# borgor/ripcurrents

Measured on AMD Instinct MI355X. Metric: frames/sec dense Farneback flow @1080p, higher is better.
Workload: dtype f32

## Files before the change

### ripcurrents_amd/csrc/flow_iter_kernels.hip

```cpp

#include <cstdlib>

#include "rc_device.h"

#define RC_ITER_BATCH 3
#define RC_RR_D 3

#ifdef RC_EXACT_BUILD
#define RC_FLOW_NS rc_flow_exact
#else
#define RC_FLOW_NS rc_flow_fast
#endif
namespace RC_FLOW_NS {

__device__ __forceinline__ float2 rc_flow_in(const RcIterArgs& a, const float2* fin, int gx, int gy) {
    if (a.in_mode == 0) return make_float2(0.f, 0.f);
    if (a.in_mode == 1) return fin[(size_t)gy * a.w + gx];
    float ax, ay;
    int sx = rc_src_x(gx, a.up_scale_x, a.fin_w, ax);
    int sx1 = min(sx + 1, a.fin_w - 1);
    int sy = rc_src_y(gy, a.up_scale_y, ay);
    int sy0 = rc_clampi(sy, 0, a.fin_h - 1), sy1 = rc_clampi(sy + 1, 0, a.fin_h - 1);
    const float2* S0 = fin + (size_t)sy0 * a.fin_w;
    const float2* S1 = fin + (size_t)sy1 * a.fin_w;
// ... 454 lines not shown
        const int g4 = idx % (TW / 4), row = (idx / (TW / 4)) % CH, c = idx / (CH * (TW / 4));
        const float4* vp = (const float4*)(V + c * CH * VP + row * VP + 4 * g4);
        float v[4 * NQ];
#pragma unroll
        for (int q = 0; q < NQ; q++) {
            float4 t = vp[q];
            v[4 * q] = t.x; v[4 * q + 1] = t.y; v[4 * q + 2] = t.z; v[4 * q + 3] = t.w;
        }
        float o[4];
#pragma unroll
        for (int p = 0; p < 4; p++) {
            float s = v[M_ + p] * a.win.k[0];
#pragma unroll
            for (int i = 1; i <= M_; i++) s += a.win.k[i] * (v[M_ + p - i] + v[M_ + p + i]);
            o[p] = s;
        }
        *(float4*)(G + c * RING * MP + row * TW + 4 * g4) = make_float4(o[0], o[1], o[2], o[3]);
    }
    __syncthreads();
    for (int px = tid; px < CH * TW; px += NT) {
        const int row = px / TW, lx = px - row * TW;
        const int gx = tx0 + lx, gy = Y + row;
        double g[5];
#pragma unroll
        for (int c = 0; c < 5; c++) g[c] = G[c * RING * MP + px];
        if (gx < a.w && gy < yend) *(float2*)(fout + (size_t)gy * a.fout_step + (size_t)gx * 8) = rc_solve(g);
    }
    __syncthreads();
}

template <int M_, int NT, int BATCH>
__global__ __launch_bounds__(NT) void k_flow_iter_sweep(RcIterArgs a) {
    using S = RcSweep<M_>;
    constexpr int CH = S::CH, MW = S::MW, MP = S::MP, RING = S::RING, TW = S::TW;
    extern __shared__ __align__(16) float smf[];
    float* ring = smf;
    float* V = smf + 5 * RING * MP;
    const int tid = threadIdx.x;
    const int z = blockIdx.y;
    const int strip = blockIdx.x % a.tiles_x, seg = blockIdx.x / a.tiles_x;
    const int tx0 = strip * TW, y0 = seg * a.th;
    const int w = a.w, h = a.h;
    const int yend = min(y0 + a.th, h);
    const size_t s0 = (size_t)((a.slot0 + z * a.zstep) % a.nslots) * a.R_slot_stride;
    const size_t s1 = (size_t)((a.slot1 + z * a.zstep) % a.nslots) * a.R_slot_stride;
    const float4* RA0 = a.RA + s0;  const float* RB0 = a.RB + s0;
    const float4* RA1 = a.RA + s1;  const float* RB1 = a.RB + s1;
    const float2* fin = a.fin ? a.fin + (size_t)z * a.fin_pair_stride : nullptr;
    char* fout = a.fout + (size_t)z * a.fout_pair_stride;

    auto matrices_rows = [&](int r0, int nrows) {
        const int n = nrows * MW;
        for (int base = tid; base < n; base += NT * BATCH) {
            float2 d[BATCH];
            int gxs[BATCH], gys[BATCH];
#pragma unroll
            for (int q = 0; q < BATCH; q++) {
                const int idx = min(base + q * NT, n - 1);
                const int j = idx / MW, lx = idx - j * MW;
                gxs[q] = rc_clampi(tx0 - M_ + lx, 0, w - 1);
                gys[q] = rc_clampi(r0 + j, 0, h - 1);
                d[q] = rc_flow_in(a, fin, gxs[q], gys[q]);
            }
            RcM5 v[BATCH];
#pragma unroll
            for (int q = 0; q < BATCH; q++)
                v[q] = rc_matrices(RA0, RB0, RA1, RB1, gxs[q], gys[q], w, h, d[q].x, d[q].y);
#pragma unroll
            for (int q = 0; q < BATCH; q++) {
                const int idx = base + q * NT;
                if (idx < n) {
                    const int j = idx / MW, lx = idx - j * MW;
                    const int slot = (r0 + j - (y0 - M_)) % RING;
                    float* mp = ring + slot * MP + lx;
                    mp[0] = v[q].m0;
                    mp[RING * MP] = v[q].m1;
                    mp[2 * RING * MP] = v[q].m2;
                    mp[3 * RING * MP] = v[q].m3;
                    mp[4 * RING * MP] = v[q].m4;
                }
            }
        }
    };
    matrices_rows(y0 - M_, 2 * M_);
    const int nsteps = (yend - y0 + CH - 1) / CH;
    for (int s = 0; s < nsteps; s++) {
        matrices_rows(y0 + M_ + CH * s, CH);
        __syncthreads();
        const int Y = y0 + CH * s;
        switch (s % (RING / CH)) {
            case 0: rc_sweep_bc<M_, NT, 0>(a, ring, V, tid, tx0, Y, yend, fout); break;
            case 1: rc_sweep_bc<M_, NT, CH>(a, ring, V, tid, tx0, Y, yend, fout); break;
            case 2: rc_sweep_bc<M_, NT, 2 * CH>(a, ring, V, tid, tx0, Y, yend, fout); break;
            default: if constexpr (RING / CH > 3) rc_sweep_bc<M_, NT, 3 * CH>(a, ring, V, tid, tx0, Y, yend, fout); break;
        }
    }
}

template <int M, int NT, int BATCH>
static void launch_iter_sweep(RcIterArgs a, int pairs, hipStream_t s) {
    using S = RcSweep<M>;
    static_assert(S::RING / S::CH <= 4, "step dispatch covers four ring phases");
    RC_ALLOW_LDS((k_flow_iter_sweep<M, NT, BATCH>), S::LDS);
    a.tw = S::TW;
    a.tiles_x = (a.w + S::TW - 1) / S::TW;
    const int want = 4 * 512;
    int segs = (want + a.tiles_x * pairs - 1) / (a.tiles_x * pairs);
    int rs = (a.h + segs - 1) / segs;
    rs = ((rs + S::CH - 1) / S::CH) * S::CH;
    if (rs < 32) rs = 32;
    a.th = rs;
    a.tiles_y = (a.h + rs - 1) / rs;
    hipLaunchKernelGGL((k_flow_iter_sweep<M, NT, BATCH>), dim3(a.tiles_x * a.tiles_y, pairs, 1), dim3(NT), S::LDS, s, a);
}

#define RC_W3_THREADS 512
template <int IN_MODE, int GAUSS_>
__global__ __launch_bounds__(RC_W3_THREADS) void k_flow_iter_w3(RcIterArgs a) {
    constexpr int TW = 64, TH = 16, MW = TW + 2, MH = TH + 2, MP = MW | 1;
    constexpr int NITEMS = MW * MH, NIT = (NITEMS + RC_W3_THREADS - 1) / RC_W3_THREADS;
    extern __shared__ __align__(16) float smf[];
    float* Ms = smf;
    const int tid = threadIdx.x;
    const int z = blockIdx.y;
    const int t = a.xcd_remap ? rc_xcd_remap(blockIdx.x, a.tiles_x * a.tiles_y) : (int)blockIdx.x;
    const int tx0 = (t % a.tiles_x) * TW, ty0 = (t / a.tiles_x) * TH;
    const int w = a.w, h = a.h;
    const size_t s0 = (size_t)((a.slot0 + z * a.zstep) % a.nslots) * a.R_slot_stride;
    const size_t s1 = (size_t)((a.slot1 + z * a.zstep) % a.nslots) * a.R_slot_stride;
    const float4* __restrict__ RA0 = a.RA + s0;  const float* __restrict__ RB0 = a.RB + s0;
    const float4* __restrict__ RA1 = a.RA + s1;  const float* __restrict__ RB1 = a.RB + s1;
    const float2* __restrict__ fin = a.fin + (size_t)z * a.fin_pair_stride;
    char* fout = a.fout + (size_t)z * a.fout_pair_stride;

    int gx[NIT], gy[NIT];
#pragma unroll
    for (int q = 0; q < NIT; q++) {
        int idx = min(tid + q * RC_W3_THREADS, NITEMS - 1);
        int ly = idx / MW, lx = idx - ly * MW;
        gx[q] = rc_clampi(tx0 - 1 + lx, 0, w - 1);
        gy[q] = rc_clampi(ty0 - 1 + ly, 0, h - 1);
    }
    float dx[NIT], dy[NIT];
    if constexpr (IN_MODE == 0) {
#pragma unroll
        for (int q = 0; q < NIT; q++) dx[q] = dy[q] = 0.f;
    } else if constexpr (IN_MODE == 1) {
        float2 d[NIT];
#pragma unroll
        for (int q = 0; q < NIT; q++) d[q] = fin[(size_t)gy[q] * w + gx[q]];
#pragma unroll
        for (int q = 0; q < NIT; q++) { dx[q] = d[q].x; dy[q] = d[q].y; }
    } else {
        float2 p00[NIT], p01[NIT], p10[NIT], p11[NIT];
        float ax[NIT], ay[NIT];
#pragma unroll
        for (int q = 0; q < NIT; q++) {
            int sx = rc_src_x(gx[q], a.up_scale_x, a.fin_w, ax[q]);
            int sx1 = min(sx + 1, a.fin_w - 1);
            int sy = rc_src_y(gy[q], a.up_scale_y, ay[q]);
            int sy0 = rc_clampi(sy, 0, a.fin_h - 1), sy1 = rc_clampi(sy + 1, 0, a.fin_h - 1);
            const float2* S0 = fin + (size_t)sy0 * a.fin_w;
            const float2* S1 = fin + (size_t)sy1 * a.fin_w;
            p00[q] = S0[sx]; p01[q] = S0[sx1]; p10[q] = S1[sx]; p11[q] = S1[sx1];
        }
#pragma unroll
        for (int q = 0; q < NIT; q++) {
            float a0 = 1.f - ax[q], a1 = ax[q], b0 = 1.f - ay[q], b1 = ay[q];
            float r0x = p00[q].x * a0 + p01[q].x * a1, r1x = p10[q].x * a0 + p11[q].x * a1;
            float r0y = p00[q].y * a0 + p01[q].y * a1, r1y = p10[q].y * a0 + p11[q].y * a1;
            dx[q] = (r0x * b0 + r1x * b1) * a.up_mul;
            dy[q] = (r0y * b0 + r1y * b1) * a.up_mul;
        }
    }
    float4 A0[NIT];
    float B0[NIT];
    RcGather gt[NIT];
#pragma unroll
    for (int q = 0; q < NIT; q++) {
        size_t p0 = (size_t)gy[q] * w + gx[q];
        A0[q] = RA0[p0];
        B0[q] = RB0[p0];
        rc_r0_prep(A0[q], B0[q]);
        rc_gather_issue(gt[q], RA1, RB1, gx[q], gy[q], dx[q], dy[q], w, h);
    }
#pragma unroll
    for (int q = 0; q < NIT; q++) {
        RcM5 v = rc_matrices_reg(A0[q], B0[q], gt[q], dx[q], dy[q], gx[q], gy[q], w, h);
        int idx = tid + q * RC_W3_THREADS;
        if (idx < NITEMS) {
            int ly = idx / MW, lx = idx - ly * MW;
            float* mp = Ms + ly * MP + lx;
            mp[0] = v.m0;
            mp[MH * MP] = v.m1;
            mp[2 * MH * MP] = v.m2;
            mp[3 * MH * MP] = v.m3;
            mp[4 * MH * MP] = v.m4;
        }
    }
    __syncthreads();

    constexpr int RPT = TH / (RC_W3_THREADS / TW);
    const int lx = tid % TW, r0 = (tid / TW) * RPT;
    const int ox = tx0 + lx;
    float g[RPT][5];
#pragma unroll
    for (int c = 0; c < 5; c++) {
        const float* mc = Ms + c * MH * MP + r0 * MP + lx;
        float col[3][RPT + 2];
#pragma unroll
        for (int j = 0; j < 3; j++)
#pragma unroll
            for (int r = 0; r < RPT + 2; r++) col[j][r] = mc[r * MP + j];
#pragma unroll
        for (int r = 0; r < RPT; r++) {
            float v[3];
#pragma unroll
            for (int j = 0; j < 3; j++) {
                if (GAUSS_) v[j] = col[j][r + 1] * a.win.k[0] + (col[j][r + 2] + col[j][r]) * a.win.k[1];
                else v[j] = col[j][r + 1] + (col[j][r + 2] + col[j][r]);
            }
            if (GAUSS_) g[r][c] = v[1] * a.win.k[0] + a.win.k[1] * (v[0] + v[2]);
            else g[r][c] = (v[1] + v[0]) + v[2];
        }
    }
    if (ox < w) {
#pragma unroll
        for (int r = 0; r < RPT; r++) {
            int oy = ty0 + r0 + r;
            if (oy < h)
                *(float2*)(fout + (size_t)oy * a.fout_step + (size_t)ox * 8) =
                    rc_solve3(g[r], GAUSS_ ? 1e-3f : (float)a.win.box_eps);
        }
    }
}

template <int IN_MODE, int G>
static void launch_w3(RcIterArgs a, int pairs, hipStream_t s) {
    a.tw = 64; a.th = 16;
    a.tiles_x = (a.w + 63) / 64; a.tiles_y = (a.h + 15) / 16;
    size_t lds = sizeof(float) * 5 * 18 * 67;
    hipLaunchKernelGGL((k_flow_iter_w3<IN_MODE, G>), dim3(a.tiles_x * a.tiles_y, pairs, 1), dim3(RC_W3_THREADS), lds, s, a);
}

template <int WW, int WH, int WP = WW>
__device__ __forceinline__ void rc_gather_window(RcGather& g, const float4* LA, const float* LB, int ox, int oy,
                                                 const float4* __restrict__ RA1, const float* __restrict__ RB1,
                                                 int gx, int gy, float dx, float dy, int w, int h) {
    float fx = gx + dx, fy = gy + dy;
    int x1 = (int)floorf(fx), y1 = (int)floorf(fy);
    g.fx = fx - x1;
    g.fy = fy - y1;
    g.inside = (unsigned)x1 < (unsigned)(w - 1) && (unsigned)y1 < (unsigned)(h - 1);
    const int wx = x1 - ox, wy = y1 - oy;
    if (g.inside && (unsigned)wx < (unsigned)(WW - 1) && (unsigned)wy < (unsigned)(WH - 1)) {
        const int i = wy * WP + wx;
        g.q00 = LA[i]; g.q01 = LA[i + 1]; g.q10 = LA[i + WP]; g.q11 = LA[i + WP + 1];
        g.e00 = LB[i]; g.e01 = LB[i + 1]; g.e10 = LB[i + WP]; g.e11 = LB[i + WP + 1];
    } else {
        const size_t p = g.inside ? (size_t)y1 * w + x1 : (size_t)gy * w + gx;
        const size_t pw = g.inside ? (size_t)w : 0, p1 = g.inside ? 1 : 0;
        g.q00 = RA1[p]; g.q01 = RA1[p + p1]; g.q10 = RA1[p + pw]; g.q11 = RA1[p + pw + p1];
        g.e00 = RB1[p]; g.e01 = RB1[p + p1]; g.e10 = RB1[p + pw]; g.e11 = RB1[p + pw + p1];
    }
}

__device__ __forceinline__ void rc_hsum3_dpp(float (&g)[5], const float (&V)[5]) {
    float t0, t1, t2, t3, t4;
    asm("s_nop 1\n\t"
        "v_add_f32_dpp %5, %10, %10 wave_shr:1 row_mask:0xf bank_mask:0xf bound_ctrl:1\n\t"
        "v_add_f32_dpp %6, %11, %11 wave_shr:1 row_mask:0xf bank_mask:0xf bound_ctrl:1\n\t"
        "v_add_f32_dpp %7, %12, %12 wave_shr:1 row_mask:0xf bank_mask:0xf bound_ctrl:1\n\t"
        "v_add_f32_dpp %8, %13, %13 wave_shr:1 row_mask:0xf bank_mask:0xf bound_ctrl:1\n\t"
        "v_add_f32_dpp %9, %14, %14 wave_shr:1 row_mask:0xf bank_mask:0xf bound_ctrl:1\n\t"
        "v_add_f32_dpp %0, %10, %5 wave_shl:1 row_mask:0xf bank_mask:0xf bound_ctrl:1\n\t"
        "v_add_f32_dpp %1, %11, %6 wave_shl:1 row_mask:0xf bank_mask:0xf bound_ctrl:1\n\t"
        "v_add_f32_dpp %2, %12, %7 wave_shl:1 row_mask:0xf bank_mask:0xf bound_ctrl:1\n\t"
        "v_add_f32_dpp %3, %13, %8 wave_shl:1 row_mask:0xf bank_mask:0xf bound_ctrl:1\n\t"
        "v_add_f32_dpp %4, %14, %9 wave_shl:1 row_mask:0xf bank_mask:0xf bound_ctrl:1"
        : "=&v"(g[0]), "=&v"(g[1]), "=&v"(g[2]), "=&v"(g[3]), "=&v"(g[4]),
          "=&v"(t0), "=&v"(t1), "=&v"(t2), "=&v"(t3), "=&v"(t4)
        : "v"(V[0]), "v"(V[1]), "v"(V[2]), "v"(V[3]), "v"(V[4]));
}


__device__ __forceinline__ void rc_hpair_dpp(float (&s)[5], const float (&V)[5]) {
    float t0, t1, t2, t3, t4;
    asm("s_nop 1\n\t"
        "v_mov_b32_dpp %5, %10 wave_shr:1 row_mask:0xf bank_mask:0xf bound_ctrl:1\n\t"
        "v_mov_b32_dpp %6, %11 wave_shr:1 row_mask:0xf bank_mask:0xf bound_ctrl:1\n\t"
        "v_mov_b32_dpp %7, %12 wave_shr:1 row_mask:0xf bank_mask:0xf bound_ctrl:1\n\t"
        "v_mov_b32_dpp %8, %13 wave_shr:1 row_mask:0xf bank_mask:0xf bound_ctrl:1\n\t"
        "v_mov_b32_dpp %9, %14 wave_shr:1 row_mask:0xf bank_mask:0xf bound_ctrl:1\n\t"
        "v_add_f32_dpp %0, %10, %5 wave_shl:1 row_mask:0xf bank_mask:0xf bound_ctrl:1\n\t"
        "v_add_f32_dpp %1, %11, %6 wave_shl:1 row_mask:0xf bank_mask:0xf bound_ctrl:1\n\t"
        "v_add_f32_dpp %2, %12, %7 wave_shl:1 row_mask:0xf bank_mask:0xf bound_ctrl:1\n\t"
        "v_add_f32_dpp %3, %13, %8 wave_shl:1 row_mask:0xf bank_mask:0xf bound_ctrl:1\n\t"
        "v_add_f32_dpp %4, %14, %9 wave_shl:1 row_mask:0xf bank_mask:0xf bound_ctrl:1"
        : "=&v"(s[0]), "=&v"(s[1]), "=&v"(s[2]), "=&v"(s[3]), "=&v"(s[4]),
          "=&v"(t0), "=&v"(t1), "=&v"(t2), "=&v"(t3), "=&v"(t4)
        : "v"(V[0]), "v"(V[1]), "v"(V[2]), "v"(V[3]), "v"(V[4]));
}

template <int GAUSS_, int NIT, int MW, int NG>
__device__ __forceinline__ void rc_rr_flows(const float (&m)[NIT][5], const float* XR, int grp, int x,
                                            const RcWindow& win, float2 (&f)[NIT]) {
    const int gu = max(grp - 1, 0), gd = min(grp + 1, NG - 1);
    const int bu = (int)__umul24((unsigned)gu, 10u * MW) + x, bd = (int)__umul24((unsigned)gd, 10u * MW) + x;
    float up[5], dn[5];
#pragma unroll
    for (int c = 0; c < 5; c++) {
        up[c] = XR[bu + (5 + c) * MW];
        dn[c] = XR[bd + c * MW];
    }
    float V[NIT][5];
#pragma unroll
    for (int q = 0; q < NIT; q++)
#pragma unroll
        for (int c = 0; c < 5; c++) {
            float u = q > 0 ? m[q - 1][c] : up[c], d = q < NIT - 1 ? m[q + 1][c] : dn[c];
            if (GAUSS_) V[q][c] = m[q][c] * win.k[0] + (d + u) * win.k[1];
            else V[q][c] = m[q][c] + (d + u);
        }
#pragma unroll
    for (int q = 0; q < NIT; q++) {
        float g[5];
        if (GAUSS_) {
            float lr[5];
            rc_hpair_dpp(lr, V[q]);
#pragma unroll
            for (int c = 0; c < 5; c++) g[c] = V[q][c] * win.k[0] + win.k[1] * lr[c];
        } else {
            rc_hsum3_dpp(g, V[q]);
        }
        f[q] = rc_solve3(g, GAUSS_ ? 1e-3f : (float)win.box_eps);
    }
}

template <int NIT, int MW>
__device__ __forceinline__ void rc_rr_exchange(const float (&m)[NIT][5], float* XR, int grp, int x) {
    const int b = (int)__umul24((unsigned)grp, 10u * MW) + x;
#pragma unroll
    for (int c = 0; c < 5; c++) {
        XR[b + c * MW] = m[0][c];
        XR[b + (5 + c) * MW] = m[NIT - 1][c];
    }
}

template <int IN_MODE, int NIT, int MW, int MH, bool INTERIOR = false>
__device__ __forceinline__ void rc_rr_flow_in(const RcIterArgs& a, const float2* __restrict__ fin, int tx0, int ty0,
                                              int gxo, const int (&gys)[NIT], float (&dx)[NIT], float (&dy)[NIT]) {
    const int w = a.w, h = a.h;
    if constexpr (IN_MODE == 0) {
#pragma unroll
        for (int q = 0; q < NIT; q++) dx[q] = dy[q] = 0.f;
    } else if constexpr (IN_MODE == 1) {
        float2 d[NIT];
#pragma unroll
        for (int q = 0; q < NIT; q++) d[q] = INTERIOR ? fin[(unsigned)(gys[q] * w + gxo)] : fin[(size_t)gys[q] * w + gxo];
#pragma unroll
        for (int q = 0; q < NIT; q++) { dx[q] = d[q].x; dy[q] = d[q].y; }
    } else if ((NIT % 2 == 0) && a.up_exact2 && (INTERIOR || (ty0 - 2 >= 0 && ty0 - 2 + MH <= h))) {
        constexpr int NR = NIT / 2 + 2;
        int sx = (gxo - 1) >> 1;
        float ax = (gxo & 1) ? 0.25f : 0.75f;
        if (!INTERIOR) {
            if (sx < 0) { ax = 0.f; sx = 0; }
            if (sx >= a.fin_w - 1) { ax = 0.f; sx = a.fin_w - 1; }
        }
        const int sx1 = min(sx + 1, a.fin_w - 1);
        const int rb = (gys[0] - 1) >> 1;
        float2 t0[NR], t1[NR];
        typedef float rc_f4a8 __attribute__((ext_vector_type(4), aligned(8)));
        const bool cols_plain = INTERIOR || (tx0 - 2 >= 1 && tx0 - 2 + MW <= w && ((tx0 - 2 + MW - 2) >> 1) + 1 <= a.fin_w - 1);
        if (INTERIOR) {
            unsigned co = (unsigned)(__mul24(rb, a.fin_w) + sx);
#pragma unroll
            for (int j = 0; j < NR; j++) {
                const rc_f4a8 v = *(const rc_f4a8*)(fin + co);
                t0[j] = make_float2(v.x, v.y); t1[j] = make_float2(v.z, v.w);
                co += (unsigned)a.fin_w;
            }
        } else if (cols_plain) {
#pragma unroll
            for (int j = 0; j < NR; j++) {
                const float2* S = fin + (size_t)rc_clampi(rb + j, 0, a.fin_h - 1) * a.fin_w;
                const rc_f4a8 v = *(const rc_f4a8*)(S + sx);
                t0[j] = make_float2(v.x, v.y); t1[j] = make_float2(v.z, v.w);
            }
        } else {
#pragma unroll
            for (int j = 0; j < NR; j++) {
                const float2* S = fin + (size_t)rc_clampi(rb + j, 0, a.fin_h - 1) * a.fin_w;
                t0[j] = S[sx]; t1[j] = S[sx1];
            }
        }
        const float a0 = 1.f - ax, a1 = ax;
        float hx[NR], hy[NR];
#pragma unroll
        for (int j = 0; j < NR; j++) {
            hx[j] = t0[j].x * a0 + t1[j].x * a1;
            hy[j] = t0[j].y * a0 + t1[j].y * a1;
        }
#pragma unroll
        for (int q = 0; q < NIT; q++) {
            const int j0 = (q + 1) >> 1;
            const float b1 = (q & 1) ? 0.25f : 0.75f, b0 = 1.f - b1;
            dx[q] = (hx[j0] * b0 + hx[j0 + 1] * b1) * a.up_mul;
            dy[q] = (hy[j0] * b0 + hy[j0 + 1] * b1) * a.up_mul;
        }
    } else {
        float2 p00[NIT], p01[NIT], p10[NIT], p11[NIT];
        float ax, ay[NIT];
        int sx, sys[NIT];
        if (a.up_exact2) {
            sx = (gxo - 1) >> 1;
            ax = (gxo & 1) ? 0.25f : 0.75f;
            if (sx < 0) { ax = 0.f; sx = 0; }
            if (sx >= a.fin_w - 1) { ax = 0.f; sx = a.fin_w - 1; }
#pragma unroll
            for (int q = 0; q < NIT; q++) { sys[q] = (gys[q] - 1) >> 1; ay[q] = (gys[q] & 1) ? 0.25f : 0.75f; }
        } else {
            sx = rc_src_x(gxo, a.up_scale_x, a.fin_w, ax);
#pragma unroll
            for (int q = 0; q < NIT; q++) sys[q] = rc_src_y(gys[q], a.up_scale_y, ay[q]);
        }
        const int sx1 = min(sx + 1, a.fin_w - 1);
#pragma unroll
        for (int q = 0; q < NIT; q++) {
            int sy = sys[q];
            int sy0 = rc_clampi(sy, 0, a.fin_h - 1), sy1 = rc_clampi(sy + 1, 0, a.fin_h - 1);
            const float2* S0 = fin + (size_t)sy0 * a.fin_w;
            const float2* S1 = fin + (size_t)sy1 * a.fin_w;
            p00[q] = S0[sx]; p01[q] = S0[sx1]; p10[q] = S1[sx]; p11[q] = S1[sx1];
        }
#pragma unroll
        for (int q = 0; q < NIT; q++) {
            float a0 = 1.f - ax, a1 = ax, b0 = 1.f - ay[q], b1 = ay[q];
            float r0x = p00[q].x * a0 + p01[q].x * a1, r1x = p10[q].x * a0 + p11[q].x * a1;
            float r0y = p00[q].y * a0 + p01[q].y * a1, r1y = p10[q].y * a0 + p11[q].y * a1;
            dx[q] = (r0x * b0 + r1x * b1) * a.up_mul;
            dy[q] = (r0y * b0 + r1y * b1) * a.up_mul;
        }
    }
}


__device__ __forceinline__ void rc_lds_barrier() { asm volatile("s_waitcnt lgkmcnt(0)\n\ts_barrier" ::: "memory"); }
__device__ __forceinline__ void rc_all_barrier() { asm volatile("s_waitcnt vmcnt(0) lgkmcnt(0)\n\ts_barrier" ::: "memory"); }

constexpr bool rc_recip_exact(int nt, int wp) {
    const unsigned r = (65536u + wp - 1) / wp;
    for (int t = 0; t < nt; t++)
        if ((int)((t * r) >> 16) != t / wp) return false;
    return true;
}

__device__ __forceinline__ void rc_glds16_s(const void* base, unsigned voff, uint32_t lds_wave_addr) {
    asm volatile("s_mov_b32 m0, %2\n\ts_nop 0\n\tglobal_load_lds_dwordx4 %0, %1" ::"v"(voff), "s"(base), "s"(lds_wave_addr) : "memory");
}
__device__ __forceinline__ void rc_glds4_s(const void* base, unsigned voff, uint32_t lds_wave_addr) {
    asm volatile("s_mov_b32 m0, %2\n\ts_nop 0\n\tglobal_load_lds_dword %0, %1" ::"v"(voff), "s"(base), "s"(lds_wave_addr) : "memory");
}

template <bool INTERIOR, int NT, int WP, int WN, int NWL>
__device__ __forceinline__ void rc_rrc_issue_window(const float4* __restrict__ RA1, const float* __restrict__ RB1,
                                                    uint32_t lds_a, uint32_t lds_b, int tid, int ox, int oy, int w, int h) {
    constexpr int QY = NT / WP, QX = NT % WP;
    const int wave_base = __builtin_amdgcn_readfirstlane(tid & ~63);
    static_assert(rc_recip_exact(NT, WP), "tid / WP by multiply and shift must be exact for every thread");
    int wy = (int)(__umul24((unsigned)tid, (65536u + WP - 1) / WP) >> 16), wx = tid - (int)__umul24((unsigned)wy, (unsigned)WP);
    int off = __mul24(oy + wy, w) + ox + wx;
#pragma unroll
    for (int q = 0; q < NWL; q++) {
        bool ok = (q + 1) * NT <= WN || tid + q * NT < WN;
        if (!INTERIOR) ok = ok && (unsigned)(ox + wx) < (unsigned)w && (unsigned)(oy + wy) < (unsigned)h;
        const unsigned p = ok ? (unsigned)off : 0u;
        if (q * NT + wave_base < WN) {
            rc_glds16_s(RA1, p << 4, lds_a + (uint32_t)(q * NT + wave_base) * 16u);
            rc_glds4_s(RB1, p << 2, lds_b + (uint32_t)(q * NT + wave_base) * 4u);
        }
        wx += QX; wy += QY; off += QY * w + QX;
        if (wx >= WP) { wx -= WP; wy += 1; off += w - WP; }
    }
}

template <bool INTERIOR, int NIT, int WW, int WH, int WP>
__device__ __forceinline__ void rc_rr_matrices(float (&m)[NIT][5], const float4 (&A0)[NIT], const float (&B0)[NIT],
                                               const float (&dx)[NIT], const float (&dy)[NIT], const float4* LA,
                                               const float* LB, int ox, int oy, const float4* __restrict__ RA1,
                                               const float* __restrict__ RB1, int gxo, const int (&gys)[NIT], int w, int h) {
    if constexpr (!INTERIOR) {
#pragma unroll
        for (int q = 0; q < NIT; q++) {
            RcGather g;
            rc_gather_window<WW, WH, WP>(g, LA, LB, ox, oy, RA1, RB1, gxo, gys[q], dx[q], dy[q], w, h);
            RcM5 v = rc_matrices_reg(A0[q], B0[q], g, dx[q], dy[q], gxo, gys[q], w, h, true);
            m[q][0] = v.m0; m[q][1] = v.m1; m[q][2] = v.m2; m[q][3] = v.m3; m[q][4] = v.m4;
        }
    } else {
        unsigned far = 0;
#pragma unroll
        for (int q = 0; q < NIT; q++) {
            RcGather g;
            const float fx = gxo + dx[q], fy = gys[q] + dy[q];
            const float flx = floorf(fx), fly = floorf(fy);
            const int x1 = (int)flx, y1 = (int)fly;
            g.fx = fx - flx;
            g.fy = fy - fly;
            g.inside = true;
            const int wx = x1 - ox, wy = y1 - oy;
            const bool in_win = (unsigned)wx < (unsigned)(WW - 1) && (unsigned)wy < (unsigned)(WH - 1);
            far |= in_win ? 0u : 1u << q;
            const unsigned i = in_win ? __umul24((unsigned)wy, (unsigned)WP) + (unsigned)wx : 0u;
            const float4* pa = (const float4*)((const char*)LA + (i << 4));
            const float* pb = (const float*)((const char*)LB + (i << 2));
            g.q00 = pa[0]; g.q01 = pa[1]; g.q10 = pa[WP]; g.q11 = pa[WP + 1];
            g.e00 = pb[0]; g.e01 = pb[1]; g.e10 = pb[WP]; g.e11 = pb[WP + 1];
            RcM5 v = rc_matrices_reg(A0[q], B0[q], g, dx[q], dy[q], gxo, gys[q], w, h, false);
            m[q][0] = v.m0; m[q][1] = v.m1; m[q][2] = v.m2; m[q][3] = v.m3; m[q][4] = v.m4;
        }
        if (__builtin_expect(far != 0, 0)) {
#pragma unroll
            for (int q = 0; q < NIT; q++) {
                if (far >> q & 1) {
                    RcGather g;
                    rc_gather_issue(g, RA1, RB1, gxo, gys[q], dx[q], dy[q], w, h);
                    RcM5 v = rc_matrices_reg(A0[q], B0[q], g, dx[q], dy[q], gxo, gys[q], w, h, false);
                    m[q][0] = v.m0; m[q][1] = v.m1; m[q][2] = v.m2; m[q][3] = v.m3; m[q][4] = v.m4;
                }
            }
        }
    }
}

template <bool INTERIOR, int IN_MODE, int GAUSS_, int NIT, int D, int MW, int NG>
__device__ __forceinline__ void rc_rrc_body(const RcIterArgs& a, const int zb, const int ze, float* smf, const uint32_t lds0, const int tx0, const int ty0) {
    constexpr int NT = NG * MW, MH = NG * NIT;
    constexpr int WW = MW + 2 * D, WH = MH + 2 * D, WP = WW, WN = WP * WH, NWL = (WN + NT - 1) / NT;
    constexpr int WNP = (WN + 63) & ~63;
    constexpr int MP = MW + 1, PLANE = MH * MP;
    static_assert(5 * PLANE <= 5 * WNP, "border-block M1 planes alias the R1 window");
    float4* LA = (float4*)smf;
    float* LB = smf + 4 * WNP;
    float* XR = LB + WNP;
    float* Ms = smf;
    const uint32_t lds_a = lds0, lds_b = lds0 + 16u * WNP;
    const int w = a.w, h = a.h;
    const int ox = tx0 - 2 - D, oy = ty0 - 2 - D;
#define RC_RRC_COORDS(tid_)                                                         \
    const int x = (tid_) & (MW - 1), grp = (tid_) / MW, ly0 = grp * NIT;            \
    const int px = tx0 - 2 + x;                                                     \
    const int gxo = INTERIOR ? px : rc_clampi(px, 0, w - 1);                        \
    int gys[NIT];                                                                   \
    _Pragma("unroll") for (int q = 0; q < NIT; q++)                                 \
        gys[q] = INTERIOR ? ty0 - 2 + ly0 + q : rc_clampi(ty0 - 2 + ly0 + q, 0, h - 1);

    float4 A0[NIT];
    float B0[NIT];
    float dx[NIT], dy[NIT];
    {
        const int tid = threadIdx.x;
        RC_RRC_COORDS(tid)
        const size_t s0 = (size_t)((a.slot0 + zb * a.zstep) % a.nslots) * a.R_slot_stride;
        const size_t s1 = (size_t)((a.slot1 + zb * a.zstep) % a.nslots) * a.R_slot_stride;
        rc_rrc_issue_window<INTERIOR, NT, WP, WN, NWL>(a.RA + s1, a.RB + s1, lds_a, lds_b, tid, ox, oy, w, h);
#pragma unroll
        for (int q = 0; q < NIT; q++) {
            const unsigned p0 = (unsigned)(gys[q] * w + gxo);
            A0[q] = (a.RA + s0)[p0];
            B0[q] = (a.RB + s0)[p0];
            rc_r0_prep(A0[q], B0[q]);
        }
        rc_rr_flow_in<IN_MODE, NIT, MW, MH, INTERIOR>(a, a.fin + (size_t)zb * a.fin_pair_stride, tx0, ty0, gxo, gys, dx, dy);
    }

    for (int z = zb; z < ze; z++) {
        const size_t s1 = (size_t)((a.slot1 + z * a.zstep) % a.nslots) * a.R_slot_stride;
        const float4* __restrict__ RA1 = a.RA + s1;
        const float* __restrict__ RB1 = a.RB + s1;
        const bool more = z + 1 < ze;
        int tid = threadIdx.x;
        asm volatile("" : "+v"(tid));
        RC_RRC_COORDS(tid)
        rc_all_barrier();

        float m[NIT][5];
        rc_rr_matrices<INTERIOR, NIT, WW, WH, WP>(m, A0, B0, dx, dy, LA, LB, ox, oy, RA1, RB1, gxo, gys, w, h);
        rc_rr_exchange<NIT, MW>(m, XR, grp, x);
        rc_lds_barrier();

        {
            float2 f1[NIT];
            rc_rr_flows<GAUSS_, NIT, MW, NG>(m, XR, grp, x, a.win, f1);
            float f1x[NIT], f1y[NIT];
#pragma unroll
            for (int q = 0; q < NIT; q++) { f1x[q] = f1[q].x; f1y[q] = f1[q].y; }
            rc_rr_matrices<INTERIOR, NIT, WW, WH, WP>(m, A0, B0, f1x, f1y, LA, LB, ox, oy, RA1, RB1, gxo, gys, w, h);
        }
        if (more) {
#pragma unroll
            for (int q = 0; q < NIT; q++) {
                const int i = (int)__umul24((unsigned)(gys[q] - oy), (unsigned)WP) + (gxo - ox);
                A0[q] = LA[i];
                B0[q] = LB[i];
                rc_r0_prep(A0[q], B0[q]);
            }
        }
        rc_lds_barrier();
        if constexpr (!INTERIOR) {
#pragma unroll
            for (int q = 0; q < NIT; q++)
#pragma unroll
                for (int c = 0; c < 5; c++) Ms[c * PLANE + (ly0 + q) * MP + x] = m[q][c];
            rc_lds_barrier();
#pragma unroll
            for (int q = 0; q < NIT; q++) {
                const int py = ty0 - 2 + ly0 + q;
                if ((unsigned)px >= (unsigned)w || (unsigned)py >= (unsigned)h) {
                    const int cx = gxo - (tx0 - 2), cy = gys[q] - (ty0 - 2);
#pragma unroll
                    for (int c = 0; c < 5; c++) m[q][c] = Ms[c * PLANE + cy * MP + cx];
                }
            }
        }
        rc_rr_exchange<NIT, MW>(m, XR, grp, x);
        rc_lds_barrier();

        if (more) {
            const size_t n1 = (size_t)((a.slot1 + (z + 1) * a.zstep) % a.nslots) * a.R_slot_stride;
            rc_rrc_issue_window<INTERIOR, NT, WP, WN, NWL>(a.RA + n1, a.RB + n1, lds_a, lds_b, tid, ox, oy, w, h);
        }

        {
            char* fout = a.fout + (size_t)z * a.fout_pair_stride;
            float2 f2[NIT];
            rc_rr_flows<GAUSS_, NIT, MW, NG>(m, XR, grp, x, a.win, f2);
            if (x >= 2 && x < MW - 2 && (INTERIOR || px < w)) {
                unsigned so = (unsigned)(ty0 - 2 + ly0) * (unsigned)a.fout_step + (unsigned)px * 8u;
#pragma unroll
                for (int q = 0; q < NIT; q++) {
                    const int ly = ly0 + q, py = ty0 - 2 + ly;
                    if (ly >= 2 && ly < MH - 2 && (INTERIOR || py < h)) *(float2*)(fout + so) = f2[q];
                    so += (unsigned)a.fout_step;
                }
            }
        }
        if (more) rc_rr_flow_in<IN_MODE, NIT, MW, MH, INTERIOR>(a, a.fin + (size_t)(z + 1) * a.fin_pair_stride, tx0, ty0, gxo, gys, dx, dy);
    }
#undef RC_RRC_COORDS
}

template <int IN_MODE, int GAUSS_, int NIT, int D, int MINB, int MW, int NG>
__global__ __launch_bounds__(NG * MW, MINB) void k_flow_iter2_rrc(RcIterArgs a, RcChainPlan cp) {
    constexpr int MH = NG * NIT, TW = MW - 4, TH = MH - 4;
    extern __shared__ __align__(16) float smf[];
    const int zb = cp.ngroups ? cp.start[blockIdx.y] : (int)blockIdx.y, ze = cp.ngroups ? cp.start[blockIdx.y + 1] : zb + 1;
    const int t = a.xcd_remap ? rc_xcd_remap(blockIdx.x, a.tiles_x * a.tiles_y) : (int)blockIdx.x;
    const int tx0 = (t % a.tiles_x) * TW, ty0 = (t / a.tiles_x) * TH;
    const bool interior = tx0 - 2 >= 5 && tx0 - 2 + MW <= a.w - 5 && ty0 - 2 >= 5 && ty0 - 2 + MH <= a.h - 5;
    const uint32_t lds0 = (uint32_t)(uintptr_t)(__attribute__((address_space(3))) void*)smf;
    if (interior) rc_rrc_body<true, IN_MODE, GAUSS_, NIT, D, MW, NG>(a, zb, ze, smf, lds0, tx0, ty0);
    else rc_rrc_body<false, IN_MODE, GAUSS_, NIT, D, MW, NG>(a, zb, ze, smf, lds0, tx0, ty0);
}

template <int IN_MODE, int G, int NIT, int D, int MINB, int MW = 32, int NG = 8>
static void launch_rrc_t(RcIterArgs a, const RcChainPlan& cp, int pairs, hipStream_t s) {
    constexpr int MH = NG * NIT, TW = MW - 4, TH = MH - 4;
    a.tw = TW; a.th = TH;
    a.tiles_x = (a.w + TW - 1) / TW; a.tiles_y = (a.h + TH - 1) / TH;
    constexpr int WN = (MW + 2 * D) * (MH + 2 * D), WNP = (WN + 63) & ~63;
    const size_t lds = sizeof(float) * (5 * WNP + NG * 2 * 5 * MW);
    RC_ALLOW_LDS((k_flow_iter2_rrc<IN_MODE, G, NIT, D, MINB, MW, NG>), lds);
    hipLaunchKernelGGL((k_flow_iter2_rrc<IN_MODE, G, NIT, D, MINB, MW, NG>), dim3(a.tiles_x * a.tiles_y, cp.ngroups ? cp.ngroups : pairs, 1), dim3(NG * MW), lds, s, a, cp);
}

static void rc_chain_plan(const RcIterArgs& a, int pairs, long long tiles, RcChainPlan& cp) {
    cp.ngroups = 0;
    const bool chainable = a.chain > 1 && pairs > 1 && (a.slot0 + a.zstep) % a.nslots == a.slot1 % a.nslots;
    if (!chainable) return;
    int chain = a.chain;
    if (!(a.ablate & RC_ABL_FORCE_CHAIN))
        while (chain > 1 && tiles * pairs / chain < (a.chain_min_blocks > 0 ? a.chain_min_blocks : 4096)) chain >>= 1;
    if (chain <= 1) return;
    int n = 0, z = 0;
    cp.start[0] = 0;
    while (z < pairs) {
        int left = pairs - z, c = left > chain ? chain : (left + 1) / 2;
        if (n == RC_MAX_CHAIN_GROUPS - 1) c = left;
        z += c;
        cp.start[++n] = z;
    }
    cp.ngroups = n;
}

template <int IN_MODE, int G>
static void launch_w3x2(RcIterArgs a, int pairs, hipStream_t s) {
    const long long tiles = (long long)((a.w + 27) / 28) * ((a.h + 27) / 28), blocks = tiles * pairs;
    RcChainPlan cp;
    rc_chain_plan(a, pairs, tiles, cp);
    if (cp.ngroups) launch_rrc_t<IN_MODE, G, 4, RC_RR_D, 4>(a, cp, pairs, s);
    else if (blocks < 512) launch_rrc_t<IN_MODE, G, 2, 4, 6>(a, cp, pairs, s);
    else if (blocks < 1024) launch_rrc_t<IN_MODE, G, 3, 4, 5>(a, cp, pairs, s);
    else launch_rrc_t<IN_MODE, G, 4, RC_RR_D, 4>(a, cp, pairs, s);
}

int rc_flow_iter_can_fuse2(const RcIterArgs& a) { return a.win.m == 1 && a.solve && a.addr32; }

int rc_flow_iter2_r0_reads(const RcIterArgs& a, int pairs) {
    RcChainPlan cp;
    rc_chain_plan(a, pairs, (long long)((a.w + 27) / 28) * ((a.h + 27) / 28), cp);
    return cp.ngroups ? cp.ngroups : pairs;
}

int rc_flow_chain_groups(const RcIterArgs& a, int pairs, int* starts, int cap) {
    RcChainPlan cp;
    rc_chain_plan(a, pairs, (long long)((a.w + 27) / 28) * ((a.h + 27) / 28), cp);
    for (int i = 0; i <= cp.ngroups && i < cap; i++) starts[i] = cp.start[i];
    return cp.ngroups;
}

void rc_launch_flow_iter2(const RcIterArgs& a, int pairs, hipStream_t s) {
    const int g = a.win.gaussian ? 1 : 0;
    switch (a.in_mode * 2 + g) {
        case 0: launch_w3x2<0, 0>(a, pairs, s); break;
        case 1: launch_w3x2<0, 1>(a, pairs, s); break;
        case 2: launch_w3x2<1, 0>(a, pairs, s); break;
        case 3: launch_w3x2<1, 1>(a, pairs, s); break;
        case 4: launch_w3x2<2, 0>(a, pairs, s); break;
        default: launch_w3x2<2, 1>(a, pairs, s); break;
    }
}

static size_t iter_lds(int tw, int th, int m, bool two_buffers) {
    int MW = tw + 2 * m, MH = th + 2 * m, MP = MW | 1;
    return sizeof(float) * (5 * (size_t)MH * MP + (two_buffers ? 5 * (size_t)th * MP : 0));
}

template <int TW, int TH, int M, int G>
static void launch_iter_t(RcIterArgs a, int pairs, hipStream_t s) {
    size_t lds = iter_lds(TW, TH, M, M > 1);
    RC_ALLOW_LDS((k_flow_iter<TW, TH, M, G>), lds);
    a.tw = TW; a.th = TH;
    a.tiles_x = (a.w + TW - 1) / TW; a.tiles_y = (a.h + TH - 1) / TH;
    hipLaunchKernelGGL((k_flow_iter<TW, TH, M, G>), dim3(a.tiles_x * a.tiles_y, pairs, 1), dim3(RC_BLOCK), lds, s, a);
}

static void pick_runtime_tile(int m, int& tw, int& th) {
    static const int tiles[][2] = {{64, 16}, {32, 32}, {64, 8}, {32, 16}, {16, 16}, {16, 8}, {8, 8}};
    double best = -1;
    tw = 8; th = 8;
    for (auto& t : tiles) {
        size_t lds = iter_lds(t[0], t[1], m, true);
        if (lds > 150 * 1024) continue;
        double eff = (double)(t[0] * t[1]) / ((t[0] + 2 * m) * (t[1] + 2 * m));
        if (lds > 64 * 1024) eff *= 0.6;
        if (t[0] < 64) eff *= 0.95;
        if (eff > best) { best = eff; tw = t[0]; th = t[1]; }
    }
}

void rc_launch_flow_iter(const RcIterArgs& a, int pairs, hipStream_t s) {
    const int m = a.win.m, g = a.win.gaussian ? 1 : 0;
    if (m == 1 && a.solve) {
        switch (a.in_mode * 2 + g) {
            case 0: launch_w3<0, 0>(a, pairs, s); break;
            case 1: launch_w3<0, 1>(a, pairs, s); break;
            case 2: launch_w3<1, 0>(a, pairs, s); break;
            case 3: launch_w3<1, 1>(a, pairs, s); break;
            case 4: launch_w3<2, 0>(a, pairs, s); break;
            default: launch_w3<2, 1>(a, pairs, s); break;
        }
        return;
    }
    if (m == 1) { g ? launch_iter_t<64, 16, 1, 1>(a, pairs, s) : launch_iter_t<64, 16, 1, 0>(a, pairs, s); return; }
    if (a.solve) {
        if (m == 2) { g ? launch_iter_big<2, 1, 512>(a, pairs, s) : launch_iter_big<2, 0, 512>(a, pairs, s); return; }
        const long long work = (long long)a.w * a.h * pairs;
        if (g && (m == 5 || m == 10) && !(a.ablate & RC_ABL_TILE_WINDOW) &&
            ((a.ablate & RC_ABL_FORCE_SWEEP) || work >= (m == 10 ? 900000ll : 8000000ll))) {
            m == 5 ? launch_iter_sweep<5, 1024, 1>(a, pairs, s) : launch_iter_sweep<10, 1024, 1>(a, pairs, s);
            return;
        }
        if (m == 5) { g ? launch_iter_big<5, 1, 1024>(a, pairs, s) : launch_iter_big<5, 0, 1024>(a, pairs, s); return; }
        if (m == 10) { g ? launch_iter_big<10, 1, 1024, 64>(a, pairs, s) : launch_iter_big<10, 0, 1024, 64>(a, pairs, s); return; }
    }
    if (m == 2) { g ? launch_iter_t<64, 16, 2, 1>(a, pairs, s) : launch_iter_t<64, 16, 2, 0>(a, pairs, s); return; }
    if (m == 5) { g ? launch_iter_t<32, 32, 5, 1>(a, pairs, s) : launch_iter_t<32, 32, 5, 0>(a, pairs, s); return; }
    if (m == 10) { g ? launch_iter_t<32, 32, 10, 1>(a, pairs, s) : launch_iter_t<32, 32, 10, 0>(a, pairs, s); return; }
    RcIterArgs b = a;
    pick_runtime_tile(m, b.tw, b.th);
    b.tiles_x = (b.w + b.tw - 1) / b.tw; b.tiles_y = (b.h + b.th - 1) / b.th;
    size_t lds = iter_lds(b.tw, b.th, m, true);
    RC_ALLOW_LDS((k_flow_iter<0, 0, 0, 0>), lds);
    hipLaunchKernelGGL((k_flow_iter<0, 0, 0, 0>), dim3(b.tiles_x * b.tiles_y, pairs, 1), dim3(RC_BLOCK), lds, s, b);
}

}
```

Before: 20170.

## Pair top and bottom halo row-groups into one edge wave to skip dead rows

Reassigns row groups to waves so one wave per block (rotated by block index) holds the first and last row groups, which contain the halo rows; that wave skips the second-iteration matrix rebuild for halo-only rows and the output flow for both halo rows. The other waves handle the interior groups with remapped exchange offsets in LDS. This removes redundant compute on halo rows in every iteration. It adds a second specialization of the body (more code, separate edge/non-edge templates) and reversed row indexing for the odd half of the edge wave, which can cause divergence within that wave.

```diff
diff --git a/ripcurrents_amd/csrc/flow_iter_kernels.hip b/ripcurrents_amd/csrc/flow_iter_kernels.hip
--- a/ripcurrents_amd/csrc/flow_iter_kernels.hip
+++ b/ripcurrents_amd/csrc/flow_iter_kernels.hip
@@ -780,20 +780,18 @@
         : "v"(V[0]), "v"(V[1]), "v"(V[2]), "v"(V[3]), "v"(V[4]));
 }
 
-template <int GAUSS_, int NIT, int MW, int NG>
-__device__ __forceinline__ void rc_rr_flows(const float (&m)[NIT][5], const float* XR, int grp, int x,
+template <int GAUSS_, int NIT, int MW, int Q0>
+__device__ __forceinline__ void rc_rr_flows(const float (&m)[NIT][5], const float* XR, int bu, int bd,
                                             const RcWindow& win, float2 (&f)[NIT]) {
-    const int gu = max(grp - 1, 0), gd = min(grp + 1, NG - 1);
-    const int bu = (int)__umul24((unsigned)gu, 10u * MW) + x, bd = (int)__umul24((unsigned)gd, 10u * MW) + x;
     float up[5], dn[5];
 #pragma unroll
     for (int c = 0; c < 5; c++) {
-        up[c] = XR[bu + (5 + c) * MW];
+        up[c] = Q0 == 0 ? XR[bu + c * MW] : 0.f;
         dn[c] = XR[bd + c * MW];
     }
     float V[NIT][5];
 #pragma unroll
-    for (int q = 0; q < NIT; q++)
+    for (int q = Q0; q < NIT; q++)
 #pragma unroll
         for (int c = 0; c < 5; c++) {
             float u = q > 0 ? m[q - 1][c] : up[c], d = q < NIT - 1 ? m[q + 1][c] : dn[c];
@@ -801,7 +799,7 @@
             else V[q][c] = m[q][c] + (d + u);
         }
 #pragma unroll
-    for (int q = 0; q < NIT; q++) {
+    for (int q = Q0; q < NIT; q++) {
         float g[5];
         if (GAUSS_) {
             float lr[5];
@@ -815,13 +813,12 @@
     }
 }
 
-template <int NIT, int MW>
-__device__ __forceinline__ void rc_rr_exchange(const float (&m)[NIT][5], float* XR, int grp, int x) {
-    const int b = (int)__umul24((unsigned)grp, 10u * MW) + x;
+template <bool EDGE, int NIT, int MW>
+__device__ __forceinline__ void rc_rr_exchange(const float (&m)[NIT][5], float* XR, int b0, int b1) {
 #pragma unroll
     for (int c = 0; c < 5; c++) {
-        XR[b + c * MW] = m[0][c];
-        XR[b + (5 + c) * MW] = m[NIT - 1][c];
+        if (!EDGE) XR[b0 + c * MW] = m[0][c];
+        XR[b1 + c * MW] = m[NIT - 1][c];
     }
 }
 
@@ -963,14 +960,14 @@
     }
 }
 
-template <bool INTERIOR, int NIT, int WW, int WH, int WP>
+template <bool INTERIOR, int NIT, int WW, int WH, int WP, int Q0 = 0>
 __device__ __forceinline__ void rc_rr_matrices(float (&m)[NIT][5], const float4 (&A0)[NIT], const float (&B0)[NIT],
                                                const float (&dx)[NIT], const float (&dy)[NIT], const float4* LA,
                                                const float* LB, int ox, int oy, const float4* __restrict__ RA1,
                                                const float* __restrict__ RB1, int gxo, const int (&gys)[NIT], int w, int h) {
     if constexpr (!INTERIOR) {
 #pragma unroll
-        for (int q = 0; q < NIT; q++) {
+        for (int q = Q0; q < NIT; q++) {
             RcGather g;
             rc_gather_window<WW, WH, WP>(g, LA, LB, ox, oy, RA1, RB1, gxo, gys[q], dx[q], dy[q], w, h);
             RcM5 v = rc_matrices_reg(A0[q], B0[q], g, dx[q], dy[q], gxo, gys[q], w, h, true);
@@ -979,7 +976,7 @@
     } else {
         unsigned far = 0;
 #pragma unroll
-        for (int q = 0; q < NIT; q++) {
+        for (int q = Q0; q < NIT; q++) {
             RcGather g;
             const float fx = gxo + dx[q], fy = gys[q] + dy[q];
             const float flx = floorf(fx), fly = floorf(fy);
@@ -1000,7 +997,7 @@
         }
         if (__builtin_expect(far != 0, 0)) {
 #pragma unroll
-            for (int q = 0; q < NIT; q++) {
+            for (int q = Q0; q < NIT; q++) {
                 if (far >> q & 1) {
                     RcGather g;
                     rc_gather_issue(g, RA1, RB1, gxo, gys[q], dx[q], dy[q], w, h);
@@ -1012,12 +1009,31 @@
     }
 }
 
-template <bool INTERIOR, int IN_MODE, int GAUSS_, int NIT, int D, int MW, int NG>
-__device__ __forceinline__ void rc_rrc_body(const RcIterArgs& a, const int zb, const int ze, float* smf, const uint32_t lds0, const int tx0, const int ty0) {
+template <bool EDGE, int IN_MODE, int NIT, int MW, int MH, bool INTERIOR>
+__device__ __forceinline__ void rc_rrc_flow_in(const RcIterArgs& a, const float2* __restrict__ fin, int tx0, int ty0,
+                                               int gxo, const int (&gys)[NIT], bool rev, float (&dx)[NIT], float (&dy)[NIT]) {
+    if constexpr (!EDGE || IN_MODE != 2) {
+        rc_rr_flow_in<IN_MODE, NIT, MW, MH, INTERIOR>(a, fin, tx0, ty0, gxo, gys, dx, dy);
+    } else {
+        int ga[NIT];
+        float ax[NIT], ay[NIT];
+#pragma unroll
+        for (int q = 0; q < NIT; q++) ga[q] = rev ? gys[NIT - 1 - q] : gys[q];
+        rc_rr_flow_in<IN_MODE, NIT, MW, MH, INTERIOR>(a, fin, tx0, ty0, gxo, ga, ax, ay);
+#pragma unroll
+        for (int q = 0; q < NIT; q++) { dx[q] = rev ? ax[NIT - 1 - q] : ax[q]; dy[q] = rev ? ay[NIT - 1 - q] : ay[q]; }
+    }
+}
+
+template <bool INTERIOR, bool EDGE, int IN_MODE, int GAUSS_, int NIT, int D, int MW, int NG>
+__device__ __forceinline__ void rc_rrc_body(const RcIterArgs& a, const int zb, const int ze, float* smf, const uint32_t lds0,
+                                            const int tx0, const int ty0, const int g0) {
     constexpr int NT = NG * MW, MH = NG * NIT;
     constexpr int WW = MW + 2 * D, WH = MH + 2 * D, WP = WW, WN = WP * WH, NWL = (WN + NT - 1) / NT;
     constexpr int WNP = (WN + 63) & ~63;
     constexpr int MP = MW + 1, PLANE = MH * MP;
+    constexpr int Q1 = EDGE ? 1 : 0, Q2 = EDGE ? 2 : 0;
+    static_assert(2 * MW == 64 && NG % 2 == 0 && NG >= 4 && NIT >= 2, "two groups per wave, the edge groups are halo + output rows");
     static_assert(5 * PLANE <= 5 * WNP, "border-block M1 planes alias the R1 window");
     float4* LA = (float4*)smf;
     float* LB = smf + 4 * WNP;
@@ -1027,12 +1043,20 @@
     const int w = a.w, h = a.h;
     const int ox = tx0 - 2 - D, oy = ty0 - 2 - D;
 #define RC_RRC_COORDS(tid_)                                                         \
-    const int x = (tid_) & (MW - 1), grp = (tid_) / MW, ly0 = grp * NIT;            \
+    const int x = (tid_) & (MW - 1);                                                \
+    const bool odd = ((tid_) & MW) != 0;                                            \
     const int px = tx0 - 2 + x;                                                     \
     const int gxo = INTERIOR ? px : rc_clampi(px, 0, w - 1);                        \
-    int gys[NIT];                                                                   \
-    _Pragma("unroll") for (int q = 0; q < NIT; q++)                                 \
-        gys[q] = INTERIOR ? ty0 - 2 + ly0 + q : rc_clampi(ty0 - 2 + ly0 + q, 0, h - 1);
+    const int grp = g0 + (odd ? 1 : 0);                                             \
+    int lys[NIT], gys[NIT];                                                         \
+    _Pragma("unroll") for (int q = 0; q < NIT; q++) {                               \
+        lys[q] = EDGE ? (odd ? MH - 1 - q : q) : grp * NIT + q;                     \
+        gys[q] = INTERIOR ? ty0 - 2 + lys[q] : rc_clampi(ty0 - 2 + lys[q], 0, h - 1); \
+    }                                                                               \
+    const int xr0 = (int)__umul24((unsigned)grp, 10u * MW) + x;                     \
+    const int xr1 = EDGE ? (odd ? (NG - 1) * 10 * MW : 5 * MW) + x : xr0 + 5 * MW;  \
+    const int xu = xr0 - 5 * MW;                                                    \
+    const int xd = EDGE ? (odd ? ((NG - 2) * 10 + 5) * MW : 10 * MW) + x : xr0 + 10 * MW;
 
     float4 A0[NIT];
     float B0[NIT];
@@ -1040,6 +1064,7 @@
     {
         const int tid = threadIdx.x;
         RC_RRC_COORDS(tid)
+        (void)xr1; (void)xu; (void)xd;
         const size_t s0 = (size_t)((a.slot0 + zb * a.zstep) % a.nslots) * a.R_slot_stride;
         const size_t s1 = (size_t)((a.slot1 + zb * a.zstep) % a.nslots) * a.R_slot_stride;
         rc_rrc_issue_window<INTERIOR, NT, WP, WN, NWL>(a.RA + s1, a.RB + s1, lds_a, lds_b, tid, ox, oy, w, h);
@@ -1050,7 +1075,7 @@
             B0[q] = (a.RB + s0)[p0];
             rc_r0_prep(A0[q], B0[q]);
         }
-        rc_rr_flow_in<IN_MODE, NIT, MW, MH, INTERIOR>(a, a.fin + (size_t)zb * a.fin_pair_stride, tx0, ty0, gxo, gys, dx, dy);
+        rc_rrc_flow_in<EDGE, IN_MODE, NIT, MW, MH, INTERIOR>(a, a.fin + (size_t)zb * a.fin_pair_stride, tx0, ty0, gxo, gys, odd, dx, dy);
     }
 
     for (int z = zb; z < ze; z++) {
@@ -1065,16 +1090,16 @@
 
         float m[NIT][5];
         rc_rr_matrices<INTERIOR, NIT, WW, WH, WP>(m, A0, B0, dx, dy, LA, LB, ox, oy, RA1, RB1, gxo, gys, w, h);
-        rc_rr_exchange<NIT, MW>(m, XR, grp, x);
+        rc_rr_exchange<EDGE, NIT, MW>(m, XR, xr0, xr1);
         rc_lds_barrier();
 
         {
             float2 f1[NIT];
-            rc_rr_flows<GAUSS_, NIT, MW, NG>(m, XR, grp, x, a.win, f1);
+            rc_rr_flows<GAUSS_, NIT, MW, Q1>(m, XR, xu, xd, a.win, f1);
             float f1x[NIT], f1y[NIT];
 #pragma unroll
-            for (int q = 0; q < NIT; q++) { f1x[q] = f1[q].x; f1y[q] = f1[q].y; }
-            rc_rr_matrices<INTERIOR, NIT, WW, WH, WP>(m, A0, B0, f1x, f1y, LA, LB, ox, oy, RA1, RB1, gxo, gys, w, h);
+            for (int q = 0; q < NIT; q++) { f1x[q] = q < Q1 ? 0.f : f1[q].x; f1y[q] = q < Q1 ? 0.f : f1[q].y; }
+            rc_rr_matrices<INTERIOR, NIT, WW, WH, WP, Q1>(m, A0, B0, f1x, f1y, LA, LB, ox, oy, RA1, RB1, gxo, gys, w, h);
         }
         if (more) {
 #pragma unroll
@@ -1088,13 +1113,13 @@
         rc_lds_barrier();
         if constexpr (!INTERIOR) {
 #pragma unroll
-            for (int q = 0; q < NIT; q++)
-#pragma unroll
-                for (int c = 0; c < 5; c++) Ms[c * PLANE + (ly0 + q) * MP + x] = m[q][c];
+            for (int q = Q1; q < NIT; q++)
+#pragma unroll
+                for (int c = 0; c < 5; c++) Ms[c * PLANE + lys[q] * MP + x] = m[q][c];
             rc_lds_barrier();
 #pragma unroll
-            for (int q = 0; q < NIT; q++) {
-                const int py = ty0 - 2 + ly0 + q;
+            for (int q = Q1; q < NIT; q++) {
+                const int py = ty0 - 2 + lys[q];
                 if ((unsigned)px >= (unsigned)w || (unsigned)py >= (unsigned)h) {
                     const int cx = gxo - (tx0 - 2), cy = gys[q] - (ty0 - 2);
 #pragma unroll
@@ -1102,7 +1127,7 @@
                 }
             }
         }
-        rc_rr_exchange<NIT, MW>(m, XR, grp, x);
+        rc_rr_exchange<EDGE, NIT, MW>(m, XR, xr0, xr1);
         rc_lds_barrier();
 
         if (more) {
@@ -1110,21 +1135,21 @@
             rc_rrc_issue_window<INTERIOR, NT, WP, WN, NWL>(a.RA + n1, a.RB + n1, lds_a, lds_b, tid, ox, oy, w, h);
         }
 
-        {
+        if constexpr (Q2 < NIT) {
             char* fout = a.fout + (size_t)z * a.fout_pair_stride;
             float2 f2[NIT];
-            rc_rr_flows<GAUSS_, NIT, MW, NG>(m, XR, grp, x, a.win, f2);
+            rc_rr_flows<GAUSS_, NIT, MW, Q2>(m, XR, xu, xd, a.win, f2);
             if (x >= 2 && x < MW - 2 && (INTERIOR || px < w)) {
-                unsigned so = (unsigned)(ty0 - 2 + ly0) * (unsigned)a.fout_step + (unsigned)px * 8u;
-#pragma unroll
-                for (int q = 0; q < NIT; q++) {
-                    const int ly = ly0 + q, py = ty0 - 2 + ly;
-                    if (ly >= 2 && ly < MH - 2 && (INTERIOR || py < h)) *(float2*)(fout + so) = f2[q];
-                    so += (unsigned)a.fout_step;
+                unsigned so = (unsigned)(ty0 - 2 + lys[Q2]) * (unsigned)a.fout_step + (unsigned)px * 8u;
+                const unsigned sstep = EDGE && odd ? 0u - (unsigned)a.fout_step : (unsigned)a.fout_step;
+#pragma unroll
+                for (int q = Q2; q < NIT; q++) {
+                    if (INTERIOR || ty0 - 2 + lys[q] < h) *(float2*)(fout + so) = f2[q];
+                    so += sstep;
                 }
             }
         }
-        if (more) rc_rr_flow_in<IN_MODE, NIT, MW, MH, INTERIOR>(a, a.fin + (size_t)(z + 1) * a.fin_pair_stride, tx0, ty0, gxo, gys, dx, dy);
+        if (more) rc_rrc_flow_in<EDGE, IN_MODE, NIT, MW, MH, INTERIOR>(a, a.fin + (size_t)(z + 1) * a.fin_pair_stride, tx0, ty0, gxo, gys, odd, dx, dy);
     }
 #undef RC_RRC_COORDS
 }
@@ -1138,8 +1163,17 @@
     const int tx0 = (t % a.tiles_x) * TW, ty0 = (t / a.tiles_x) * TH;
     const bool interior = tx0 - 2 >= 5 && tx0 - 2 + MW <= a.w - 5 && ty0 - 2 >= 5 && ty0 - 2 + MH <= a.h - 5;
     const uint32_t lds0 = (uint32_t)(uintptr_t)(__attribute__((address_space(3))) void*)smf;
-    if (interior) rc_rrc_body<true, IN_MODE, GAUSS_, NIT, D, MW, NG>(a, zb, ze, smf, lds0, tx0, ty0);
-    else rc_rrc_body<false, IN_MODE, GAUSS_, NIT, D, MW, NG>(a, zb, ze, smf, lds0, tx0, ty0);
+    const int wv = __builtin_amdgcn_readfirstlane((int)threadIdx.x) >> 6;
+    const int ew = (int)(blockIdx.x + blockIdx.y) & (NG / 2 - 1);
+    static_assert((NG / 2 & (NG / 2 - 1)) == 0, "edge wave by mask");
+    const int g0 = 1 + 2 * (wv - (wv > ew ? 1 : 0));
+    if (wv == ew) {
+        if (interior) rc_rrc_body<true, true, IN_MODE, GAUSS_, NIT, D, MW, NG>(a, zb, ze, smf, lds0, tx0, ty0, 0);
+        else rc_rrc_body<false, true, IN_MODE, GAUSS_, NIT, D, MW, NG>(a, zb, ze, smf, lds0, tx0, ty0, 0);
+    } else {
+        if (interior) rc_rrc_body<true, false, IN_MODE, GAUSS_, NIT, D, MW, NG>(a, zb, ze, smf, lds0, tx0, ty0, g0);
+        else rc_rrc_body<false, false, IN_MODE, GAUSS_, NIT, D, MW, NG>(a, zb, ze, smf, lds0, tx0, ty0, g0);
+    }
 }
 
 template <int IN_MODE, int G, int NIT, int D, int MINB, int MW = 32, int NG = 8>
```

After: 20300 (median of 6 runs). About the same (+0.7%).
